# JiaxuanYou/graph-pooling

Measured on AMD Instinct MI355X. Metric: graphs/sec fwd+bwd, DD padded batch N_max=500, higher is better.
Workload: dtype f32; 1 GPU; S-DD: DD-shaped padded batch, B=20/GPU, N_max=500, F=89, H=E=20, K=50, L=3, 1 pool; graphs_per_gpu=20, global_batch=20, linkpred=False, hip_graph=True, parallelism=dp1

## Files before the change

### graph_pooling_amd/csrc/dp_common.h

```cpp
#pragma once
#include <hip/hip_runtime.h>
#include <cstddef>
#include <cstdint>
#include <cstdio>
#include <cstring>
#include <atomic>
#include <mutex>

#include "../../include/diffpool_hip.h"

namespace dp {

void set_error(const char* fmt, ...);
const char* last_error();

#define DP_CHECK_ARG(cond, ...)                      \
    do {                                             \
        if (!(cond)) {                               \
            ::dp::set_error(__VA_ARGS__);            \
            return DP_ERR_INVALID_ARG;               \
        }                                            \
    } while (0)

int* device_error_word();
// ... 413 lines not shown
    const float* x0[2];
    int x_shared;
    const float* params;
    L0Stack st[2];
    const float* Y[DP_MAX_LAYERS];
    const float* invn[DP_MAX_LAYERS];
    const float* stats[DP_MAX_LAYERS];
    const float* Z[2];
    int ldz[2];
    int coff[2][DP_MAX_LAYERS];
    int K;
    long wp_off, bp_off;
    const float* S;
    const float* Tt;
    const float* dXn;
    const float* dAn;
    const float* d_assign;
    const float* dZe;
    const unsigned short *pkA, *pkAt;
    int pk_ld;
    const int* pk_flag;
    const int* pk_sym;
    float* slabs;
    long slab_gstride;
    unsigned short* vs;
    float* part;
    float* gpart;
    int* bar;
};
bool level0_bwd_persistent_ok(const Level0Bwd& a);
size_t level0_bwd_vs_elems(const Level0Bwd& a);
size_t level0_bwd_gpart_floats(const Level0Bwd& a);
void level0_backward(Seq& q, const Level0Bwd& a);
bool level0_persistent_ok(const Level0Fwd& a);
size_t level0_bar_ints(int B);
int* level0_seq_word(int* bar);
size_t level0_xpart_floats(const Level0Fwd& a);
size_t level0_vs_elems(const Level0Fwd& a);
size_t level0_part_floats(const Level0Fwd& a);
size_t level0_mpart_floats(const Level0Fwd& a);
const int* level0_error_word(const int* bar);
void level0_forward(Seq& q, const Level0Fwd& a);

struct HeadArgs {
    const float* Z;
    int ldz, n, rw, featoff;
    int* argmax;
    int lda;
    const float* params;
    int n_pred;
    int dims[DP_MAX_PRED + 2];
    long w_off[DP_MAX_PRED + 1], b_off[DP_MAX_PRED + 1];
    float* hid[DP_MAX_PRED + 2];
    int B;
    long long* labels;
    const int* poison[DP_MAX_LEVELS + 1];
    int n_poison;
};
struct HeadBwdArgs {
    HeadArgs h;
    const float* d_ypred;
    float* grads;
    int n_levels;
    struct Level {
        float* dZ;
        const int* argmax;
        int lda, n, ldz, rw, featoff;
    } lv[DP_MAX_LEVELS + 1];
};
bool head_supported(const HeadArgs& a);
void head_fwd(Seq& q, const HeadArgs& a);
void head_bwd(Seq& q, const HeadBwdArgs& a);

bool small_level_fused_ok(int B, int n, const int* dims, int L, bool dadj);
size_t small_level_part_floats(int B, int n, int L);
void small_level_fwd(Seq& q, const SmallLevelIO& io, int B, int n, const int* dims, int L, int add_self, int bn);
struct SmallHeadFold {
    HeadBwdArgs hb;
    int level;
    int zcol;
    float* part;
};
size_t small_head_fold_part_floats(const HeadArgs& h);
bool small_head_fold_fits(int B, int n, const int* dims, int L, bool dadj, const HeadArgs& h);
void small_level_bwd(Seq& q, const SmallLevelIO& io, const float* dZe, float* dX0, float* dadj, float* slabs,
                     long slab_stride, int B, int n, const int* dims, int L, int add_self, int bn,
                     const SmallHeadFold* hf = nullptr);

void build_batch(Seq& q, const int* src, const int* dst, const int* edge_ptr, const int* label, const int* node_ptr,
                 float* adj, unsigned short* pk, unsigned short* pkt, float* feats, float* assign, int* num_nodes,
                 int* errors, int* degree, int B, int N, int F, int mode, int symmetric, int max_edges_per_graph);

void gather_labels(Seq& q, const long long* src, long long* dst, int B);

void clip_adam_step(Seq& q, float* params, float* grads, float* exp_avg, float* exp_avg_sq, long n, float max_norm,
                    float beta1, float beta2, float eps, float step_size, float inv_bc2_sqrt, float* total_norm_out,
                    int* step_counter = nullptr, float lr = 0.f);

void csr_aggregate_fwd(Seq& q, const float* table, int ldt, const int* indptr, const int* indices, float* out, int ldo,
                       int n_rows, int feat, int mean, float beta, const float* values = nullptr);
void csr_aggregate_bwd_scatter(Seq& q, const float* dout, int ldo, const int* indptr, const int* indices, float* dtable,
                               int ldt, int n_rows, int feat, int mean, const float* values = nullptr);

void segment_max_part(Seq& q, const float* Z, int ldz, const int* chunk_tab, int n_chunks, int F, float* pv, int* pi);

void set2set_prep_weights(Seq& q, const float* w_ih, const float* w_hh, float* wt, int d);

void linkpred_fwd(Seq& q, const float* S, int lds, const float* adj, const int* num_nodes, float* loss_out,
                  int B, int n, int K, const float* norm = nullptr );
void linkpred_bwd(Seq& q, const float* S, int lds, const float* adj, const int* num_nodes, const float* dloss,
                  float* dS, int ldds, int B, int n, int K, int accumulate, const float* norm = nullptr);
void linkpred_fwd_packed(Seq& q, const float* S, int lds, const unsigned short* pk, const int* num_nodes,
                         float* loss_out, int B, int n, int K, const float* norm = nullptr);
void linkpred_bwd_packed(Seq& q, const float* S, int lds, const unsigned short* pk, const unsigned short* pkt,
                         const int* num_nodes, const float* dloss, float* dS, int ldds, int B, int n, int K,
                         int accumulate, const float* norm = nullptr);

struct AssignEntPick {
    int lanes;
    int quad;
};
AssignEntPick assign_ent_pick(const void* S, int lds, const void* dS, int ldds, int K);
size_t assign_ent_part_doubles();
void assign_entropy_fwd(Seq& q, const float* S, int lds, const int* num_nodes, float weight, float* ent_out,
                        float* total_inout, int B, int n, int K);
void assign_entropy_bwd(Seq& q, const float* S, int lds, const int* num_nodes, const float* dloss, float weight,
                        float* dS, int ldds, int accumulate, int B, int n, int K);

size_t frob_link_ws_doubles(long long rows, int B, int K);
void frob_link_w_dense(Seq& q, const float* S, int lds, const void* adj, const void* adj_t, int packed, int ld,
                       const int* num_nodes, float* W, int B, int N, int K);
void frob_link_fwd(Seq& q, const float* S, int lds, const float* W, const void* adj, int adj_kind, int adj_ld,
                   const int* num_nodes, const int* node_off, const int* nnz_ptr, const float* link_norm, float wscale,
                   float* G, float* loss_out, float* total_inout, int B, int N, long long rows, int K,
                   const int* csr_indptr = nullptr );
void frob_link_bwd(Seq& q, const float* S, int lds, const float* W, const float* G, const int* num_nodes,
                   const int* node_off, const float* link_norm, const float* dloss, float wscale, float* dS, int ldds,
                   int accumulate, int B, int N, long long rows, int K);

}
```

### graph_pooling_amd/csrc/dp_model.hip

```cpp
#include "dp_common.h"

namespace dp {

void set2set_fwd(Seq& q, const float* emb, int lde, const float* w_ih, const float* w_hh, const float* b_ih,
                 const float* b_hh, const float* Wp, const float* bp, float* out, int B, int n, int d, void* save);
void set2set_bwd(Seq& q, const float* emb, int lde, const float* w_ih, const float* w_hh, const float* b_ih,
                 const float* b_hh, const float* Wp, const float* bp, const float* out, const float* dout,
                 float* demb, int ldde, float* dw_ih, float* dw_hh, float* db_ih, float* db_hh, float* dWp,
                 float* dbp, int B, int n, int d, const void* save);
size_t set2set_save_bytes(int B, int n, int d);

namespace {

struct LevelInfo {
    int j;
    int n, G, L;
    const dp_stack_cfg* e;
    const dp_stack_cfg* a;
    int D, Da, K;
    int ctot[DP_MAX_LAYERS];
    int coff_e[DP_MAX_LAYERS], coff_a[DP_MAX_LAYERS];
    int cmax;
};

// ... 1135 lines not shown
                featoff += rw;
            } else {
                set2set_bwd(q, sv.Zm, li.D, PW(params, c.s2s_off[0]), PW(params, c.s2s_off[1]), PW(params, c.s2s_off[2]),
                            PW(params, c.s2s_off[3]), PW(params, c.s2s_off[4]), PW(params, c.s2s_off[5]), sv.feat, dfeat,
                            dZm, li.D, grads + c.s2s_off[0], grads + c.s2s_off[1], grads + c.s2s_off[2],
                            grads + c.s2s_off[3], grads + c.s2s_off[4], grads + c.s2s_off[5], B, li.n, li.D, sv.s2s);
                mask_rows(q, dZm, li.D, gr[j].dZe, li.D, num_nodes, B, li.n, li.D);
            }
        }
    }
    for (int j = P; j >= 0; --j) {
        const LevelInfo& li = p.lv[j];
        const LevelSave& lv = sv.lv[j];
        const int n = li.n;
        if (p.bwd[j] == Tier::Persistent) {
            Level0Bwd f = p.l0b;
            level0_operands(f, sv, params, x, adj, assign_x);
            f.dXn = P >= 1 ? gr[1].dX0 : nullptr;
            f.dAn = P >= 1 ? gr[1].dAdj : nullptr;
            f.d_assign = d_assign;
            f.dZe = gr[0].dZe;
            f.slabs = slabs;
            f.slab_gstride = slab_stride * KS;
            f.vs = l0_vs; f.part = wh.xr.l0_bwd; f.gpart = l0_gpart;
            f.bar = wh.l0_bar;
            level0_backward(q, f);
            continue;
        }
        LevelIO io = level_io(j, sv, x, adj, assign_x, dropout, sc, pkp);
        if (j < P) {
            const int K = li.K, D = li.D;
            float *const dS = sc.dS, *const dlog = sc.dlog, *const V = sc.V, *const V2 = sc.V2;
            unsigned short* const vs = sc.vs;
            bool vsplit_used = false;
            const float* dS2 = nullptr;
            const float* dXn = gr[j + 1].dX0;
            const float* dAn = gr[j + 1].dAdj;
            {
                unsigned short* vsplit =
                    (j == 0 && pkp && aggregate_packed_usable(io.adj, n, K)) ? vs : nullptr;
                vsplit_used = vsplit != nullptr;
                GemmDesc d[4] = {
                    {lv.S, dXn, gr[j].dZe, nullptr, n, D, K, K, D, D, (long)n * K, (long)K * D, (long)n * D, false, false,
                     1.f, 1.f, 0},
                    {lv.Ze, dXn, dS, nullptr, n, K, D, D, D, K, (long)n * D, (long)K * D, (long)n * K, false, true, 1.f,
                     0.f, 0},
                    {lv.S, dAn, V, nullptr, n, K, K, K, K, K, (long)n * K, (long)K * K, (long)n * K, false, true, 1.f, 0.f,
                     0, 0, 0, vsplit, (K + 15) / 16, ((n + 31) / 32) * 4, 0},
                    {lv.S, dAn, V2, nullptr, n, K, K, K, K, K, (long)n * K, (long)K * K, (long)n * K, false, false, 1.f,
                     0.f, 0}};
                if (!gr[j].dAdj) {
                    d[3] = GemmDesc{lv.T, dAn, V2, nullptr, n, K, K, K, K, K, (long)n * K, (long)K * K, (long)n * K, false,
                                    false, 1.f, 0.f, 0};
                    dS2 = V2;
                }
                bgemm_group(q, d, 4, B);
            }
            if (gr[j].dAdj)
                bgemm(q, lv.T, dAn, dS, nullptr, B, n, K, K, K, K, K, (long)n * K, (long)K * K, (long)n * K, false, false,
                      1.f, 1.f, 0);
            aggregate(q, io.adj, V, K, dS, K, B, n, K, false, 1.f, j == 0 ? pkp : nullptr, vs, vsplit_used);
            if (gr[j].dAdj)
                bgemm(q, V2, lv.S, gr[j].dAdj, nullptr, B, n, n, K, K, K, n, (long)n * K, (long)n * K, (long)n * n, false,
                      true, 1.f, 1.f, 0);
            if (j == 0 && d_assign) axpy(q, dS, d_assign, 1.f, (long)B * n * K);
            softmax_mask_bwd(q, lv.S, K, dS, K, j == 0 ? num_nodes : nullptr, dlog, K, B, n, K,
                             c.assign_pred_b_off[j] >= 0 ? slabs + c.assign_pred_b_off[j] : nullptr, slab_stride * KS,
                             dS2);
            {
                const int ksn = n >= 256 ? KS : 1;
                GemmDesc d2[2] = {
                    {dlog, lv.Za, slabs + c.assign_pred_w_off[j], nullptr, K, li.Da, n, K, li.Da, li.Da, (long)n * K,
                     (long)n * li.Da, slab_stride * KS, true, false, 1.f, 0.f, 0, slab_stride, 0},
                    {dlog, PW(params, c.assign_pred_w_off[j]), gr[j].dZa, nullptr, n, li.Da, K, K, li.Da, li.Da,
                     (long)n * K, 0, (long)n * li.Da, false, false, 1.f, 0.f, 0, 0, 0, nullptr, 0, 0, 0, 1}};
                bgemm_group(q, d2, 2, B, ksn);
            }
        }
        io.bar = bz.bar + 64 * j;
        io.gr = &gr[j];
        io.hf = fold && j == P ? &hf : nullptr;
        level_backward(q, p, j, lv, io, params, sc);
    }
    reduce_slabs(q, slabs, slab_stride, B * KS, grads, c.n_graph_params, 0);
    return q.err;
}

size_t encoder_save_bytes(const dp_encoder_cfg& c) { return layout_save(encoder_plan(c, false), nullptr).total; }

int encoder_save_locate(const dp_encoder_cfg& c, int level, int field, size_t* offset, size_t* count) {
    char* const base = reinterpret_cast<char*>(size_t(1) << 20);
    const EncoderPlan plan = encoder_plan(c, false);
    SaveLayout sv = layout_save(plan, base);
    const LevelInfo& li = plan.lv[level];
    const LevelSave& lv = sv.lv[level];
    const size_t B = c.B;
    const void* p = nullptr;
    size_t cnt = 0;
    switch (field) {
        case DP_SAVE_ARGMAX: p = lv.argmax; cnt = B * readout_width(c, li); break;
        case DP_SAVE_S: p = lv.S; cnt = B * li.n * li.K; break;
        case DP_SAVE_XPOOL: p = lv.Xn; cnt = B * li.K * li.D; break;
        case DP_SAVE_ADJPOOL: p = lv.An; cnt = B * li.K * li.K; break;
        case DP_SAVE_Z: p = lv.Ze; cnt = B * li.n * li.D; break;
        case DP_SAVE_ZASSIGN: p = lv.Za; cnt = B * li.n * li.Da; break;
        default: set_error("dp_encoder_save_locate: unknown field %d", field); return DP_ERR_INVALID_ARG;
    }
    if (!p) {
        set_error("dp_encoder_save_locate: level %d has no field %d", level, field);
        return DP_ERR_INVALID_ARG;
    }
    *offset = (size_t)(static_cast<const char*>(p) - base);
    *count = cnt;
    return DP_OK;
}

int encoder_validate(const dp_encoder_cfg* c) { return validate(c); }

}
```

### graph_pooling_amd/csrc/dp_rowops.hip

```cpp
#include "dp_common.h"

namespace dp {

#define L2_EPS 1e-12f
#define BN_EPS 1e-5f

typedef float f4u __attribute__((ext_vector_type(4), aligned(4)));

__device__ inline float team_sum(float v) {
    return row16_sum(v);
}
__device__ inline float team_max(float v) {
    return row16_max(v);
}

static inline bool row_quads_ok(const RowGroups& g) {
    if (knobs().no_row_quads) return false;
    for (int i = 0; i < g.G; ++i)
        if (g.w[i] < 4 || (g.w[i] & 3)) return false;
    return true;
}
static inline int team_grid(long items) {
    long blocks = (items + 15) / 16;
    if (blocks > 4096) blocks = 4096;
// ... 1800 lines not shown
void relu_bwd_inplace(Seq& q, float* d, const float* h, long count) {
    if (!q.ok() || count <= 0) return;
    hipLaunchKernelGGL(k_relu_bwd, dim3((count + 255) / 256), dim3(256), 0, q.stream, d, h, count);
    q.check_launch("relu_bwd");
}

__global__ void k_axpy(float* y, const float* x, float a, long count) {
    const long i = (long)blockIdx.x * blockDim.x + threadIdx.x;
    if (i < count) y[i] += a * x[i];
}
void axpy(Seq& q, float* y, const float* x, float a, long count) {
    if (!q.ok() || count <= 0) return;
    hipLaunchKernelGGL(k_axpy, dim3((count + 255) / 256), dim3(256), 0, q.stream, y, x, a, count);
    q.check_launch("axpy");
}

__global__ __launch_bounds__(256) void k_ce_fwd(const float* logits, const long long* label, float* loss,
                                                float* prob, int B, int C, float* also_zero, float* dunit) {
    __shared__ float red[256];
    float acc = 0.f;
    for (int b = threadIdx.x; b < B; b += 256) {
        const float* l = logits + (long)b * C;
        float m = -INFINITY;
        for (int c = 0; c < C; ++c) m = fmaxf(m, l[c]);
        float s = 0.f;
        for (int c = 0; c < C; ++c) s += expf(l[c] - m);
        const float lse = m + logf(s);
        const long long y = label[b];
        acc += lse - l[y];
        if (prob)
            for (int c = 0; c < C; ++c) prob[(long)b * C + c] = expf(l[c] - lse);
        if (dunit)
            for (int c = 0; c < C; ++c)
                dunit[(long)b * C + c] = (expf(l[c] - lse) - (y == c ? 1.f : 0.f)) / (float)B;
    }
    red[threadIdx.x] = acc;
    __syncthreads();
    for (int s = 128; s > 0; s >>= 1) {
        if (threadIdx.x < s) red[threadIdx.x] += red[threadIdx.x + s];
        __syncthreads();
    }
    if (threadIdx.x == 0) {
        loss[0] = red[0] / (float)B;
        if (also_zero) also_zero[0] = 0.f;
    }
}
void ce_fwd(Seq& q, const float* logits, const long long* label, float* loss, float* prob, int B, int C,
            float* also_zero, float* dunit) {
    if (!q.ok()) return;
    hipLaunchKernelGGL(k_ce_fwd, dim3(1), dim3(256), 0, q.stream, logits, label, loss, prob, B, C, also_zero, dunit);
    q.check_launch("ce_fwd");
}
__global__ void k_ce_bwd(const float* prob, const long long* label, const float* dloss, float scale, float* dl,
                         int B, int C) {
    const int i = blockIdx.x * blockDim.x + threadIdx.x;
    if (i >= B * C) return;
    const int b = i / C, c = i % C;
    const float g = (dloss ? dloss[0] : 1.f) * scale / (float)B;
    dl[i] = g * (prob[i] - (label[b] == c ? 1.f : 0.f));
}
void ce_bwd(Seq& q, const float* prob, const long long* label, const float* dloss, float scale, float* dlogits,
            int B, int C) {
    if (!q.ok()) return;
    hipLaunchKernelGGL(k_ce_bwd, dim3((B * C + 255) / 256), dim3(256), 0, q.stream, prob, label, dloss, scale,
                       dlogits, B, C);
    q.check_launch("ce_bwd");
}

__global__ void k_argmax_rows(const float* X, int ldx, long long* out, int rows, int cols) {
    const int r = blockIdx.x * blockDim.x + threadIdx.x;
    if (r >= rows) return;
    const float* x = X + (long)r * ldx;
    int best = 0;
    for (int c = 1; c < cols; ++c)
        if (x[c] > x[best]) best = c;
    out[r] = best;
}
void argmax_rows(Seq& q, const float* X, int ldx, long long* out, int rows, int cols) {
    if (!q.ok() || rows <= 0) return;
    hipLaunchKernelGGL(k_argmax_rows, dim3((rows + 255) / 256), dim3(256), 0, q.stream, X, ldx, out, rows, cols);
    q.check_launch("argmax_rows");
}

__global__ __launch_bounds__(1024) void k_reduce_slabs(const float* slabs, long stride, int B, float* out,
                                                       long count, int accumulate) {
    __shared__ float red[16][64];
    const int cl = threadIdx.x & 63, rl = threadIdx.x >> 6;
    const long i = (long)blockIdx.x * 64 + cl;
    float s = 0.f;
    if (i < count)
        for (int b = rl; b < B; b += 16) s += slabs[(long)b * stride + i];
    red[rl][cl] = s;
    __syncthreads();
    if (rl == 0 && i < count) {
        float t = 0.f;
#pragma unroll
        for (int k = 0; k < 16; ++k) t += red[k][cl];
        out[i] = accumulate ? out[i] + t : t;
    }
}
void reduce_slabs(Seq& q, const float* slabs, long stride, int B, float* out, long count, int accumulate) {
    if (!q.ok() || count <= 0) return;
    hipLaunchKernelGGL(k_reduce_slabs, dim3((count + 63) / 64), dim3(1024), 0, q.stream, slabs, stride, B, out, count,
                       accumulate);
    q.check_launch("reduce_slabs");
}

}
```

### graph_pooling_amd/csrc/dp_small.hip

```cpp
#include "dp_common.h"

namespace dp {

#define SM_L2_EPS 1e-12f
#define SM_BN_EPS 1e-5f

#ifdef DP_STAMP
__device__ unsigned long long g_small_stamps[2][32];
#define SM_STAMP(k, i)                                                                       \
    do {                                                                                     \
        if (blockIdx.x == 0 && threadIdx.x == 0) g_small_stamps[k][i] = __builtin_amdgcn_s_memtime(); \
    } while (0)
#else
#define SM_STAMP(k, i) \
    do {               \
    } while (0)
#endif

namespace {

__device__ inline float sm_team_sum(float v) {
    return row16_sum(v);
}

// ... 547 lines not shown
                if (tl == 0) sc_st16(part_l, (unsigned)(((long)r * a.B + b) * 16), sc_tagged(mean, m2, (seq << 4) | (unsigned)(l + 1)));
            }
        }
        SM_STAMP(0, 12 + 6 * l);
        if (last) break;
        if (stats) {
            SM_STAMP(0, 13 + 6 * l);
            for (int r = team; r < n; r += NTEAMS) {
                float pm[SM_BMAX16], pq[SM_BMAX16];
                const bool ok = sm_poll_row(part_l, (unsigned)((long)r * a.B * 16), a.B, bn_tag, pm, pq, a.spin_limit, a.bar,
                                            a.dev_err);
                float sm = 0.f;
#pragma unroll
                for (int u = 0; u < SM_BMAX16; ++u) sm += (tl + 16 * u < a.B) ? pm[u] : 0.f;
                float m = sm_team_sum(sm) / (float)a.B;
                float s2 = 0.f;
#pragma unroll
                for (int u = 0; u < SM_BMAX16; ++u) {
                    const float d = pm[u] - m;
                    s2 += (tl + 16 * u < a.B) ? pq[u] + (float)dout * d * d : 0.f;
                }
                float rstd = 1.0f / sqrtf(sm_team_sum(s2) / ((float)a.B * (float)dout) + SM_BN_EPS);
                if (!ok) m = rstd = __builtin_nanf("");
                if (tl == 0) {
                    if (b == 0) {
                        a.stats[l][r * 2] = m;
                        a.stats[l][r * 2 + 1] = rstd;
                    }
                    mu[r] = m;
                    rs[r] = rstd;
                }
            }
            SM_STAMP(0, 14 + 6 * l);
        } else {
            for (int r = tid; r < n; r += NT) {
                mu[r] = 0.f;
                rs[r] = 1.f;
            }
        }
        lds_barrier();
        for (int r = team; r < n; r += NTEAMS)
            for (int k = tl; k < dout; k += 16) {
                const float v = (fmaxf(U[r * dout + k], 0.f) - mu[r]) * rs[r];
                X[r * dout + k] = v;
                a.Ze[((long)b * n + r) * a.ldz + a.coff[l] + k] = v;
            }
        lds_barrier();
        SM_STAMP(0, 15 + 6 * l);
        wo += din * dout;
        bo += dout;
    }
    sm_finish(a.bar, a.seq, seq, a.B);
}

struct SmallLevelBwdArgs {
    const float* adj;
    const float* x0;
    int ldx0;
    const float* params;
    long w_off[DP_MAX_LAYERS], b_off[DP_MAX_LAYERS];
    int dims[DP_MAX_LAYERS + 1];
    int L;
    const float* Y[DP_MAX_LAYERS];
    int ldY[DP_MAX_LAYERS];
    const float* invn[DP_MAX_LAYERS];
    const float* stats[DP_MAX_LAYERS];
    const float* Ze;
    int ldz;
    int coff[DP_MAX_LAYERS];
    const float* dZe;
    float* dX0;
    float* dadj;
    float* slabs;
    long slab_stride;
    float* part;
    int* bar;
    int* seq;
    int* dev_err;
    int spin_limit, target_bias;
    int B, n, add_self, bn;
    int omax, wtot, D;
    SmDiv qd0, qD;
    SmDiv qdout[DP_MAX_LAYERS];
    int fold, hlevel, zcol, htot;
    HeadBwdArgs hb;
    float* hpart;
};

struct SmHead {
    int nP, d0, d1, C, wup, hup, E;
    __host__ __device__ SmHead(const HeadArgs& h) : nP(h.n_pred), d0(h.dims[0]), d1(h.dims[1]), C(h.dims[h.n_pred]) {
        wup = hup = 0;
        for (int i = 1; i < nP; ++i) {
            wup += h.dims[i] * h.dims[i + 1];
            hup += h.dims[i];
        }
        E = (hup + 1) / 2;
    }
    __host__ __device__ size_t lds_floats(int B) const {
        return (size_t)d1 * d0 + wup + 2 * (size_t)B * hup + (size_t)B * d0 + (size_t)B * C;
    }
};
constexpr unsigned SM_HEAD_TAG = 15u;

__global__ __launch_bounds__(1024) void k_small_level_bwd(SmallLevelBwdArgs a) {
    extern __shared__ __attribute__((aligned(16))) float lds[];
    const int b = blockIdx.x, tid = threadIdx.x;
    const int n = a.n, L = a.L, D = a.D, d0 = a.dims[0];
    const unsigned seq = (unsigned)a.seq[0];
    float* A = lds;
    float* DA = A + n * n;
    float* X0 = DA + (a.dadj ? n * n : 0);
    float* ZE = X0 + n * d0;
    float* DZ = ZE + n * D;
    float* YS = DZ + n * D;
    float* WL = YS + (L - 1) * n * a.omax;
    float* IV = WL + a.wtot;
    float* RS = IV + L * n;
    float* dU = RS + L * n;
    float* G = dU + n * a.omax;
    float* P = G + n * a.omax;
    float* M0 = P + n * a.omax;
    float* M1 = M0 + n;
    float* DB = M1 + n;
    float* DBW = DB + a.omax;
    const int tl = tid & 15, team = tid >> 4;
    const int NT = blockDim.x, NTEAMS = blockDim.x >> 4;
    const SmHead hz(a.hb.h);
    const int B = a.B;
    float* HW0 = DBW + 16 * a.omax;
    float* HWU = HW0 + hz.d1 * hz.d0;
    float* HH = HWU + hz.wup;
    float* HG = HH + B * hz.hup;
    float* HF = HG + B * hz.hup;
    float* HY = HF + B * hz.d0;
    SM_STAMP(1, 16);
    int win = -1;
    if (a.fold) {
        if (tid < hz.d0) {
            for (int lv = 0; lv < a.hb.n_levels; ++lv) {
                const int f = tid - a.hb.lv[lv].featoff;
                if (f >= 0 && f < a.hb.lv[lv].rw) win = a.hb.lv[lv].argmax[(long)b * a.hb.lv[lv].lda + f];
            }
        }
        const HeadArgs& h = a.hb.h;
        sm_dma(HY, B * hz.C, [&](int e) { return a.hb.d_ypred + e; });
        sm_dma(HW0, hz.d1 * hz.d0, [&](int e) { return h.params + h.w_off[0] + e; });
        int wo = 0, ho = 0;
        for (int i = 1; i < hz.nP; ++i) {
            const int cnt = h.dims[i] * h.dims[i + 1];
            sm_dma(HWU + wo, cnt, [&](int e) { return h.params + h.w_off[i] + e; });
            sm_dma(HH + ho, B * h.dims[i], [&](int e) { return h.hid[i] + e; });
            wo += cnt;
            ho += B * h.dims[i];
        }
        sm_dma(HF, B * hz.d0, [&](int e) { return h.hid[0] + e; });
    }

    sm_dma(A, n * n, [&](int e) { return a.adj + (long)b * n * n + e; });
    sm_dma(X0, n * d0, [&](int e) { return a.x0 + ((long)b * n + a.qd0.quot(e)) * a.ldx0 + a.qd0.rem(e); });
    sm_dma(ZE, n * D, [&](int e) { return a.Ze + ((long)b * n + a.qD.quot(e)) * a.ldz + a.qD.rem(e); });
    sm_dma(DZ, n * D, [&](int e) { return a.dZe + ((long)b * n + a.qD.quot(e)) * a.ldz + a.qD.rem(e); });
    {
        int wo = 0;
        for (int l = 0; l < L; ++l) {
            const int din = a.dims[l], dout = a.dims[l + 1];
            const float* w = a.params + a.w_off[l];
            sm_dma(WL + wo, din * dout, [&](int e) { return w + e; });
            wo += din * dout;
            const float* iv = a.invn[l] + (long)b * n;
            sm_dma(IV + l * n, n, [&](int e) { return iv + e; });
            if (l < L - 1) {
                const float* y = a.Y[l];
                const int ldy = a.ldY[l];
                const SmDiv q = a.qdout[l];
                sm_dma(YS + l * n * a.omax, n * dout, [&](int e) { return y + ((long)b * n + q.quot(e)) * ldy + q.rem(e); });
                if (a.bn) {
                    const float* st = a.stats[l];
                    sm_dma(RS + l * n, n, [&](int e) { return st + e * 2 + 1; });
                }
            }
        }
    }
    if (a.dadj)
        for (int i = tid; i < n * n; i += NT) DA[i] = 0.f;
    SM_STAMP(1, 17);
    __syncthreads();
    SM_STAMP(1, 18);

    if (a.fold) {
        const HeadArgs& h = a.hb.h;
        int ho = B * hz.hup, wo = hz.wup;
        for (int i = hz.nP - 1; i >= 1; --i) {
            const int din = h.dims[i], dout = h.dims[i + 1];
            wo -= din * dout;
            ho -= B * din;
            const float* go = i == hz.nP - 1 ? HY + b * dout : HG + ho + B * din + b * dout;
            const float* W = HWU + wo;
            for (int k = tid; k < din; k += NT) {
                float s = 0.f;
#pragma unroll 8
                for (int j = 0; j < dout; ++j) s += go[j] * W[j * din + k];
                HG[ho + b * din + k] = HH[ho + b * din + k] > 0.f ? s : 0.f;
            }
            __syncthreads();
        }
        const ScBuf hp = sc_buf(a.hpart, (size_t)B * hz.E * 16);
        for (int e = tid; e < hz.E; e += NT) {
            float v[2] = {0.f, 0.f};
            for (int u = 0; u < 2; ++u) {
                int t = 2 * e + u, blk = 0;
                for (int i = 1; i < hz.nP && t >= 0; ++i) {
                    if (t < h.dims[i]) v[u] = HG[blk + b * h.dims[i] + t];
                    t -= h.dims[i];
                    blk += B * h.dims[i];
                }
            }
            sc_st16(hp, (unsigned)(((long)b * hz.E + e) * 16), sc_tagged(v[0], v[1], (seq << 4) | SM_HEAD_TAG));
        }
        const float* g1 = hz.nP == 1 ? HY + b * hz.C : HG + b * hz.d1;
        for (int k = tid, it = 0; k < hz.d0; k += NT, ++it) {
            float s = 0.f;
#pragma unroll 8
            for (int j = 0; j < hz.d1; ++j) s += g1[j] * HW0[j * hz.d0 + k];
            for (int lv = 0; lv < a.hb.n_levels; ++lv) {
                const HeadBwdArgs::Level& t = a.hb.lv[lv];
                const int f = k - t.featoff;
                if (f >= 0 && f < t.rw) {
                    const int r = it == 0 ? win : t.argmax[(long)b * t.lda + f];
                    if (r < 0) continue;
                    if (lv == a.hlevel) DZ[r * D + a.zcol + f] += s;
                    else t.dZ[((long)b * t.n + r) * t.ldz + f] = s;
                }
            }
        }
        SM_STAMP(1, 19);
    }

    u32x4 hprobe = (u32x4){0u, 0u, 0u, 0u};
    const unsigned htag = ((seq << 4) | SM_HEAD_TAG) ^ (a.target_bias ? 0x40000000u : 0u);
    int wo_end = a.wtot;
    for (int l = L - 1; l >= 0; --l) {
        const int din = a.dims[l], dout = a.dims[l + 1];
        const bool last = l == L - 1;
        const bool has_bn = !last && a.bn;
        const bool has_relu = !last;
        wo_end -= din * dout;
        const float* W = WL + wo_end;
        const float* Xl = l == 0 ? X0 : ZE + a.coff[l - 1];
        const int ldx = l == 0 ? d0 : D;
        const float* Yl = last ? ZE + a.coff[l] : YS + l * n * a.omax;
        const int ldy = last ? D : dout;
        float* dx = DZ + a.coff[l];
        for (int i = tid; i < 16 * dout; i += NT) DBW[i] = 0.f;
        if (has_bn) {
            const ScBuf part_l = sc_buf(a.part + (long)l * a.B * n * 4, (size_t)a.B * n * 16);
            const unsigned bn_tag = (seq << 4) | (unsigned)(l + 1);
            const float* xh = ZE + a.coff[l];
            for (int r = team; r < n; r += NTEAMS) {
                float s0 = 0.f, s1 = 0.f;
                for (int c = tl; c < dout; c += 16) {
                    const float d = dx[r * D + c];
                    s0 += d;
                    s1 += d * xh[r * D + c];
                }
                s0 = sm_team_sum(s0);
                s1 = sm_team_sum(s1);
                if (tl == 0) sc_st16(part_l, (unsigned)(((long)r * a.B + b) * 16), sc_tagged(s0, s1, bn_tag));
            }
            for (int r = team; r < n; r += NTEAMS) {
                float p0[SM_BMAX16], p1[SM_BMAX16];
                const bool ok = sm_poll_row(part_l, (unsigned)((long)r * a.B * 16), a.B,
                                            bn_tag ^ (a.target_bias ? 0x40000000u : 0u), p0, p1, a.spin_limit, a.bar, a.dev_err);
                float s0 = 0.f, s1 = 0.f;
#pragma unroll
                for (int u = 0; u < SM_BMAX16; ++u) {
                    s0 += (tl + 16 * u < a.B) ? p0[u] : 0.f;
                    s1 += (tl + 16 * u < a.B) ? p1[u] : 0.f;
                }
                s0 = sm_team_sum(s0);
                s1 = sm_team_sum(s1);
                const float cnt = (float)a.B * (float)dout;
                if (tl == 0) {
                    M0[r] = ok ? s0 / cnt : __builtin_nanf("");
                    M1[r] = s1 / cnt;
                }
            }
        }
        if (a.fold && l == 0 && tid < B * hz.E) hprobe = sc_ld16(sc_buf(a.hpart, (size_t)B * hz.E * 16), (unsigned)tid * 16u);
        lds_barrier();
        float* dbb = a.b_off[l] >= 0 ? a.slabs + (long)b * a.slab_stride + a.b_off[l] : nullptr;
        for (int r0 = 0; r0 < n; r0 += NTEAMS) {
            const int r = min(r0 + team, n - 1);
            const bool valid = r0 + team < n;
            const float rstd = has_bn ? RS[l * n + r] : 1.f;
            const float m0 = has_bn ? M0[r] : 0.f, m1 = has_bn ? M1[r] : 0.f;
            const float inv = IV[l * n + r];
            const bool project = inv < 1.0f / SM_L2_EPS;
            float dot = 0.f;
            float dv[4];
#pragma unroll
            for (int k = 0; k < 4; ++k) {
                const int c = tl + 16 * k;
                float d = 0.f;
                if (c < dout) {
                    d = dx[r * D + c];
                    const float yy = Yl[r * ldy + c];
                    if (has_bn) d = rstd * (d - m0 - ZE[r * D + a.coff[l] + c] * m1);
                    if (has_relu) d = yy > 0.f ? d : 0.f;
                    dot += d * yy;
                }
                dv[k] = d;
            }
            dot = sm_team_sum(dot);
#pragma unroll
            for (int k = 0; k < 4; ++k) {
                const int c = tl + 16 * k;
                float v = 0.f;
                if (c < dout && valid) {
                    v = project ? inv * (dv[k] - Yl[r * ldy + c] * dot) : inv * dv[k];
                    dU[r * dout + c] = v;
                }
                if (dbb && 16 * k < dout) {
                    v += __shfl_xor(v, 16, 64);
                    v += __shfl_xor(v, 32, 64);
                    if ((tid & 63) < 16 && c < dout) DBW[(tid >> 6) * dout + c] += v;
                }
            }
        }
        lds_barrier();
        if (dbb)
            for (int c = tid; c < dout; c += NT) {
                float t = 0.f;
#pragma unroll
                for (int w = 0; w < 16; ++w) t += DBW[w * dout + c];
                dbb[c] = t;
            }
        lds_mma2<true, false>(A, n, dU, dout, n, dout, n, [&](int m, int c, float v) {
            G[m * dout + c] = a.add_self ? v + dU[m * dout + c] : v;
        });
        if (a.dadj)
            lds_mma2<false, false>(Xl, ldx, W, dout, n, dout, din, [&](int m, int c, float v) { P[m * dout + c] = v; },
                                  ((n + 15) / 16) * ((dout + 15) / 16));
        lds_barrier();
        {
            float* dWb = a.slabs + (long)b * a.slab_stride + a.w_off[l];
            lds_mma2<true, false>(Xl, ldx, G, dout, din, dout, n, [&](int k, int c, float v) { dWb[k * dout + c] = v; });
        }
        if (l > 0) {
            float* dxin = DZ + a.coff[l - 1];
            lds_mma2<false, true>(G, dout, W, dout, n, din, dout, [&](int r, int k, float v) { dxin[r * D + k] += v; },
                                 1);
        } else if (a.dX0) {
            lds_mma2<false, true>(G, dout, W, dout, n, din, dout, [&](int r, int k, float v) {
                a.dX0[((long)b * n + r) * d0 + k] = v;
            }, 1);
        }
        if (a.dadj)
            lds_mma2<false, true>(dU, dout, P, dout, n, n, dout, [&](int r, int m, float v) { DA[r * n + m] += v; }, 2);
        lds_barrier();
    }
    if (a.dadj)
        for (int i = tid; i < n * n; i += NT) a.dadj[(long)b * n * n + i] = DA[i];
    SM_STAMP(1, 20);
    if (a.fold) {
        const HeadArgs& h = a.hb.h;
        const ScBuf hp = sc_buf(a.hpart, (size_t)B * hz.E * 16);
        bool ok = true;
        for (int t = tid; t < B * hz.E; t += NT) {
            const int bb = t / hz.E, e = t - bb * hz.E;
            u32x4 q = hprobe;
            for (int it = 0;; ++it) {
                if (t != tid || it > 0) q = sc_ld16(hp, (unsigned)t * 16u);
                if (q[1] == htag && q[3] == htag) break;
                if (it > a.spin_limit) {
                    __hip_atomic_store(a.bar + 1, 1, __ATOMIC_RELAXED, __HIP_MEMORY_SCOPE_AGENT);
                    dev_err_raise(a.dev_err, DP_DEVERR_BARRIER);
                    ok = false;
                    break;
                }
                if (t != tid || it > 0) __builtin_amdgcn_s_sleep(2);
            }
            for (int u = 0; u < 2; ++u) {
                int x = 2 * e + u, blk = 0;
                for (int i = 1; i < hz.nP && x >= 0; ++i) {
                    if (x < h.dims[i]) HG[blk + bb * h.dims[i] + x] = __uint_as_float(q[2 * u]);
                    x -= h.dims[i];
                    blk += B * h.dims[i];
                }
            }
        }
        ok = __syncthreads_and(ok);
        SM_STAMP(1, 21);
        const int lo = a.htot * b / B, hi = a.htot * (b + 1) / B;
        for (int e = lo + tid; e < hi; e += NT) {
            int i = 0, r = e, ho = 0;
            for (; i < hz.nP - 1; ++i) {
                const int seg = h.dims[i + 1] * (h.dims[i] + (h.b_off[i] >= 0 ? 1 : 0));
                if (r < seg) break;
                r -= seg;
                if (i > 0) ho += B * h.dims[i];
            }
            const int din = h.dims[i], dout = h.dims[i + 1];
            const float* go = i == hz.nP - 1 ? HY : HG + (i > 0 ? ho + B * din : 0);
            const float* hin = i == 0 ? HF : HH + ho;
            float s = 0.f;
            if (r < dout * din) {
                const int j = r / din, k = r - j * din;
#pragma unroll 8
                for (int bb = 0; bb < B; ++bb) s += go[bb * dout + j] * hin[bb * din + k];
                a.hb.grads[h.w_off[i] + r] = ok ? s : __builtin_nanf("");
            } else {
                const int j = r - dout * din;
#pragma unroll 8
                for (int bb = 0; bb < B; ++bb) s += go[bb * dout + j];
                a.hb.grads[h.b_off[i] + j] = ok ? s : __builtin_nanf("");
            }
        }
        SM_STAMP(1, 22);
    }
    sm_finish(a.bar, a.seq, seq, a.B);
}

size_t small_lds_floats_fwd(int B, int n, int din, int dout) {
    return (size_t)n * n + (size_t)n * din + (size_t)din * dout + 2 * (size_t)n * dout + 2 * n + dout +
           (size_t)B * n * 2 + 16;
}
size_t small_lds_floats_bwd(int B, int n, int din, int dout) {
    return 2 * (size_t)n * n + 2 * (size_t)n * din + (size_t)din * dout + 4 * (size_t)n * dout + 4 * n + 17 * (size_t)dout +
           (size_t)B * n * 2 + 16;
}

}

bool small_level_supported(int B, int n, int din, int dout) {
    if (n > 64 || din > 256 || dout > 256) return false;
    const size_t f = small_lds_floats_fwd(B, n, din, dout), bw = small_lds_floats_bwd(B, n, din, dout);
    return (f > bw ? f : bw) * sizeof(float) <= 150 * 1024;
}

static void small_attr(Seq& q) {
    static DynLdsOnce fwd, bwd;
    ensure_dyn_lds(q, fwd, reinterpret_cast<const void*>(&k_small_gcn_fwd), 160 * 1024, "k_small_gcn_fwd");
    ensure_dyn_lds(q, bwd, reinterpret_cast<const void*>(&k_small_gcn_bwd), 160 * 1024, "k_small_gcn_bwd");
}

void small_gcn_fwd(Seq& q, const float* adj, const float* x0, int ldx0, const float* yprev, int ldyp,
                   const float* part_prev, float* stats_prev, float* xout, int ldxo, const float* W, const float* bias,
                   float* y, int ldy, float* invn, float* part, int B, int n, int din, int dout, int add_self,
                   int stats) {
    if (!q.ok()) return;
    small_attr(q);
    if (!q.ok()) return;
    SmallFwdArgs a{adj, x0, ldx0, yprev, ldyp, part_prev, stats_prev, xout, ldxo, W, bias, y, ldy, invn, part,
                   B, n, din, dout, add_self, stats, sm_div(din)};
    hipLaunchKernelGGL(k_small_gcn_fwd, dim3(B), dim3(1024), small_lds_floats_fwd(B, n, din, dout) * sizeof(float),
                       q.stream, a);
    q.check_launch("small_gcn_fwd");
}

void small_gcn_bwd(Seq& q, const float* adj, const float* xin, int ldxin, const float* W, const float* y, int ldy,
                   const float* xhat, int ldxh, const float* invn, const float* stats, const float* part2,
                   const float* dx, int lddx, float* dxin, int lddxin, float* part2_prev, float* dadj, float* dW,
                   float* db, long slab_stride, int B, int n, int din, int dout, int add_self, int has_bn,
                   int has_relu) {
    if (!q.ok()) return;
    small_attr(q);
    if (!q.ok()) return;
    SmallBwdArgs a{adj, xin, ldxin, W, y, ldy, xhat, ldxh, invn, stats, part2, dx, lddx, dxin, lddxin, part2_prev,
                   dadj, dW, db, slab_stride, B, n, din, dout, add_self, has_bn, has_relu, sm_div(din), sm_div(dout)};
    hipLaunchKernelGGL(k_small_gcn_bwd, dim3(B), dim3(1024), small_lds_floats_bwd(B, n, din, dout) * sizeof(float),
                       q.stream, a);
    q.check_launch("small_gcn_bwd");
}


static size_t small_level_lds_fwd(int B, int n, const int* dims, int L) {
    int dmax = 0, omax = 0, wtot = 0, btot = 0;
    for (int l = 0; l < L; ++l) {
        dmax = dims[l] > dmax ? dims[l] : dmax;
        omax = dims[l + 1] > omax ? dims[l + 1] : omax;
        wtot += dims[l] * dims[l + 1];
        btot += dims[l + 1];
    }
    return (size_t)n * n + (size_t)n * dmax + 2 * (size_t)n * omax + 2 * n + wtot + btot + 64 + 16;
}
static size_t small_level_lds_bwd(int B, int n, const int* dims, int L, bool dadj) {
    int omax = 0, wtot = 0, D = 0;
    for (int l = 0; l < L; ++l) {
        omax = dims[l + 1] > omax ? dims[l + 1] : omax;
        wtot += dims[l] * dims[l + 1];
        D += dims[l + 1];
    }
    return (size_t)n * n * (dadj ? 2 : 1) + (size_t)n * dims[0] + 2 * (size_t)n * D + (size_t)(L - 1) * n * omax + wtot +
           2 * (size_t)L * n + 3 * (size_t)n * omax + 2 * n + 17 * (size_t)omax + 64 + 16;
}
static int device_cus() {
    static std::atomic<int> cus[64];
    int dev = 0;
    if (hipGetDevice(&dev) != hipSuccess || dev < 0 || dev >= 64) return 0;
    int v = cus[dev].load(std::memory_order_relaxed);
    if (v == 0) {
        hipDeviceProp_t prop;
        v = hipGetDeviceProperties(&prop, dev) == hipSuccess ? prop.multiProcessorCount : -1;
        cus[dev].store(v, std::memory_order_relaxed);
    }
    return v > 0 ? v : 0;
}
static bool level_kernels_admitted() {
    static std::atomic<int> state[64];
    int dev = 0;
    if (hipGetDevice(&dev) != hipSuccess || dev < 0 || dev >= 64) return false;
    int v = state[dev].load(std::memory_order_relaxed);
    if (v == 0) {
        v = 1;
        const void* fns[2] = {reinterpret_cast<const void*>(&k_small_level_fwd),
                              reinterpret_cast<const void*>(&k_small_level_bwd)};
        for (const void* fn : fns) {
            int blocks = 0;
            hipError_t e = hipFuncSetAttribute(fn, hipFuncAttributeMaxDynamicSharedMemorySize, 159 * 1024);
            if (e == hipSuccess) e = hipOccupancyMaxActiveBlocksPerMultiprocessor(&blocks, fn, 1024, 150 * 1024);
            if (e != hipSuccess || blocks < 1) {
                (void)hipGetLastError();
                set_error("whole-level kernels disabled: the runtime admits %d resident 1024-thread workgroups with 150 KiB "
                          "of LDS per CU (%s)", blocks, hipGetErrorString(e));
                v = -1;
            }
        }
        state[dev].store(v, std::memory_order_relaxed);
    }
    return v > 0;
}
bool small_level_fused_ok(int B, int n, const int* dims, int L, bool dadj) {
    if (knobs().no_level_fusion || L < 2 || L > DP_MAX_LAYERS || n > 64) return false;
    for (int l = 0; l <= L; ++l)
        if (dims[l] > 256 || (l > 0 && dims[l] > 64)) return false;
    if (small_level_lds_fwd(B, n, dims, L) * sizeof(float) > 150 * 1024) return false;
    if (small_level_lds_bwd(B, n, dims, L, dadj) * sizeof(float) > 150 * 1024) return false;
    const int cus = device_cus();
    return cus > 0 && B <= cus / 2 && B <= 16 * SM_BMAX16 && level_kernels_admitted();
}
size_t small_level_part_floats(int B, int n, int L) { return (size_t)(L > 1 ? L - 1 : 1) * B * n * 4; }
static int head_grad_entries(const HeadArgs& h) {
    int tot = 0;
    for (int i = 0; i < h.n_pred; ++i) tot += h.dims[i + 1] * (h.dims[i] + (h.b_off[i] >= 0 ? 1 : 0));
    return tot;
}
size_t small_head_fold_part_floats(const HeadArgs& h) {
    const SmHead z(h);
    return (size_t)h.B * (z.E > 0 ? z.E : 1) * 4;
}
bool small_head_fold_fits(int B, int n, const int* dims, int L, bool dadj, const HeadArgs& h) {
    if (h.n_pred < 1 || h.B != B || (long)head_grad_entries(h) * B >= (1L << 31)) return false;
    return (small_level_lds_bwd(B, n, dims, L, dadj) + SmHead(h).lds_floats(B)) * sizeof(float) <= 150 * 1024;
}

void small_level_fwd(Seq& q, const SmallLevelIO& io, int B, int n, const int* dims, int L, int add_self, int bn) {
    if (!q.ok()) return;
    static DynLdsOnce attr;
    ensure_dyn_lds(q, attr, reinterpret_cast<const void*>(&k_small_level_fwd), 159 * 1024, "k_small_level_fwd");
    if (!q.ok()) return;
    SmallLevelFwdArgs a{};
    a.adj = io.adj; a.x0 = io.x0; a.ldx0 = io.ldx0; a.params = io.params; a.L = L;
    a.Ze = io.Ze; a.ldz = io.ldz; a.part = io.part; a.bar = io.bar; a.seq = q.seq_word;
    a.B = B; a.n = n; a.add_self = add_self; a.bn = bn;
    for (int l = 0; l <= L; ++l) a.dims[l] = dims[l];
    for (int l = 0; l < L; ++l) {
        a.w_off[l] = io.w_off[l]; a.b_off[l] = io.b_off[l];
        a.Y[l] = io.Y[l]; a.ldY[l] = io.ldY[l]; a.invn[l] = io.invn[l]; a.stats[l] = io.stats[l];
        a.coff[l] = io.coff[l];
        a.dmax = dims[l] > a.dmax ? dims[l] : a.dmax;
        a.omax = dims[l + 1] > a.omax ? dims[l + 1] : a.omax;
        a.wtot += dims[l] * dims[l + 1];
        a.btot += dims[l + 1];
    }
    a.qd0 = sm_div(dims[0]);
    a.dev_err = device_error_word();
    a.spin_limit = knobs().test_barrier_fail ? 64 : SM_SPIN_LIMIT;
    a.target_bias = knobs().test_barrier_fail ? 1 : 0;
    hipLaunchKernelGGL(k_small_level_fwd, dim3(B), dim3(1024), small_level_lds_fwd(B, n, dims, L) * sizeof(float),
                       q.stream, a);
    q.check_launch("small_level_fwd");
}

void small_level_bwd(Seq& q, const SmallLevelIO& io, const float* dZe, float* dX0, float* dadj, float* slabs,
                     long slab_stride, int B, int n, const int* dims, int L, int add_self, int bn,
                     const SmallHeadFold* hf) {
    if (!q.ok()) return;
    static DynLdsOnce attr;
    ensure_dyn_lds(q, attr, reinterpret_cast<const void*>(&k_small_level_bwd), 159 * 1024, "k_small_level_bwd");
    if (!q.ok()) return;
    SmallLevelBwdArgs a{};
    a.adj = io.adj; a.x0 = io.x0; a.ldx0 = io.ldx0; a.params = io.params; a.L = L;
    a.Ze = io.Ze; a.ldz = io.ldz; a.part = io.part; a.bar = io.bar; a.seq = q.seq_word;
    a.dZe = dZe; a.dX0 = dX0; a.dadj = dadj; a.slabs = slabs; a.slab_stride = slab_stride;
    a.B = B; a.n = n; a.add_self = add_self; a.bn = bn;
    for (int l = 0; l <= L; ++l) a.dims[l] = dims[l];
    for (int l = 0; l < L; ++l) {
        a.w_off[l] = io.w_off[l]; a.b_off[l] = io.b_off[l];
        a.Y[l] = io.Y[l]; a.ldY[l] = io.ldY[l]; a.invn[l] = io.invn[l]; a.stats[l] = io.stats[l];
        a.coff[l] = io.coff[l];
        a.omax = dims[l + 1] > a.omax ? dims[l + 1] : a.omax;
        a.wtot += dims[l] * dims[l + 1];
        a.D += dims[l + 1];
        a.qdout[l] = sm_div(dims[l + 1]);
    }
    a.qd0 = sm_div(dims[0]);
    a.qD = sm_div(a.D);
    a.dev_err = device_error_word();
    a.spin_limit = knobs().test_barrier_fail ? 64 : SM_SPIN_LIMIT;
    a.target_bias = knobs().test_barrier_fail ? 1 : 0;
    size_t lds = small_level_lds_bwd(B, n, dims, L, dadj != nullptr);
    if (hf) {
        a.fold = 1;
        a.hb = hf->hb;
        a.hlevel = hf->level;
        a.zcol = hf->zcol;
        a.hpart = hf->part;
        a.htot = head_grad_entries(hf->hb.h);
        lds += SmHead(hf->hb.h).lds_floats(B);
    }
    hipLaunchKernelGGL(k_small_level_bwd, dim3(B), dim3(1024), lds * sizeof(float), q.stream, a);
    q.check_launch("small_level_bwd");
}

#ifdef DP_STAMP
extern "C" __attribute__((visibility("default"))) int dp_debug_stamps(unsigned long long* out) {
    return (int)hipMemcpyFromSymbol(out, HIP_SYMBOL(g_small_stamps), sizeof(unsigned long long) * 64);
}
#endif

}
```

Baseline: 85420 graphs/s.

## Move head weight-gradient reduction from fused level kernel into slab-reduce kernel

The fused small-level backward kernel used to exchange per-graph head hidden gradients through tagged scratch with cross-block spin-waiting, then reduce the head weight and bias gradients over the batch inside each block. Now each block only writes its own hidden gradients to a plain buffer. The batch reduction of head gradients runs in extra workgroups appended to the final reduce_slabs launch. This removes the inter-block handshake and shrinks per-block LDS, since only one graph's head data is staged. The cost is a somewhat heavier reduce kernel that re-reads hidden activations from global memory.

```diff
diff --git a/graph_pooling_amd/csrc/dp_common.h b/graph_pooling_amd/csrc/dp_common.h
--- a/graph_pooling_amd/csrc/dp_common.h
+++ b/graph_pooling_amd/csrc/dp_common.h
@@ -519,6 +519,9 @@
     float* part;
 };
 size_t small_head_fold_part_floats(const HeadArgs& h);
+long head_grad_entries(const HeadArgs& h);
+void reduce_slabs_head(Seq& q, const float* slabs, long stride, int B, float* out, long count,
+                       const SmallHeadFold& hf);
 bool small_head_fold_fits(int B, int n, const int* dims, int L, bool dadj, const HeadArgs& h);
 void small_level_bwd(Seq& q, const SmallLevelIO& io, const float* dZe, float* dX0, float* dadj, float* slabs,
                      long slab_stride, int B, int n, const int* dims, int L, int add_self, int bn,
diff --git a/graph_pooling_amd/csrc/dp_model.hip b/graph_pooling_amd/csrc/dp_model.hip
--- a/graph_pooling_amd/csrc/dp_model.hip
+++ b/graph_pooling_amd/csrc/dp_model.hip
@@ -1241,7 +1241,8 @@
         io.hf = fold && j == P ? &hf : nullptr;
         level_backward(q, p, j, lv, io, params, sc);
     }
-    reduce_slabs(q, slabs, slab_stride, B * KS, grads, c.n_graph_params, 0);
+    if (fold) reduce_slabs_head(q, slabs, slab_stride, B * KS, grads, c.n_graph_params, hf);
+    else reduce_slabs(q, slabs, slab_stride, B * KS, grads, c.n_graph_params, 0);
     return q.err;
 }
 
diff --git a/graph_pooling_amd/csrc/dp_rowops.hip b/graph_pooling_amd/csrc/dp_rowops.hip
--- a/graph_pooling_amd/csrc/dp_rowops.hip
+++ b/graph_pooling_amd/csrc/dp_rowops.hip
@@ -1906,9 +1906,80 @@
     q.check_launch("argmax_rows");
 }
 
-__global__ __launch_bounds__(1024) void k_reduce_slabs(const float* slabs, long stride, int B, float* out,
-                                                       long count, int accumulate) {
-    __shared__ float red[16][64];
+struct HeadGradArgs {
+    int tiles;
+    int n_pred, B, hup;
+    int htot;
+    int dims[DP_MAX_PRED + 2];
+    long w_off[DP_MAX_PRED + 1], b_off[DP_MAX_PRED + 1];
+    const float* hid[DP_MAX_PRED + 1];
+    const float* d_ypred;
+    const float* hgrad;
+    float* grads;
+};
+constexpr int HG_CHUNK = 32;
+constexpr int HG_THREADS = 128;
+
+__device__ inline void head_grad_entry(const HeadGradArgs& a, int e) {
+    int i = 0, r = e, rem = e, goff = 0, gcol = 0;
+    int din = a.dims[0], dout = a.dims[1];
+    long woff = a.w_off[0], boff = a.b_off[0];
+    const float* hin = a.hid[0];
+    bool found = false;
+#pragma unroll
+    for (int t = 0; t < DP_MAX_PRED + 1; ++t) {
+        if (t < a.n_pred) {
+            const int seg = a.dims[t + 1] * (a.dims[t] + (a.b_off[t] >= 0 ? 1 : 0));
+            if (!found && (rem < seg || t == a.n_pred - 1)) {
+                i = t; r = rem; goff = gcol;
+                din = a.dims[t]; dout = a.dims[t + 1];
+                woff = a.w_off[t]; boff = a.b_off[t];
+                hin = a.hid[t];
+                found = true;
+            }
+            rem -= seg;
+            gcol += a.dims[t + 1];
+        }
+    }
+    const int B = a.B;
+    const bool weight = r < dout * din;
+    const int j = weight ? r / din : r - dout * din;
+    const int k = weight ? r - j * din : 0;
+    const bool top = i == a.n_pred - 1;
+    const float* gp = (top ? a.d_ypred : a.hgrad + goff) + j;
+    const int gs = top ? dout : a.hup;
+    const float* xp = hin + (weight ? k : 0);
+    const int xs = weight ? din : 0;
+    float s = 0.f;
+    for (int b0 = 0; b0 < B; b0 += HG_CHUNK) {
+        float g[HG_CHUNK], x[HG_CHUNK];
+#pragma unroll
+        for (int u0 = 0; u0 < HG_CHUNK; u0 += 8) {
+            if (b0 + u0 < B) {
+#pragma unroll
+                for (int u = u0; u < u0 + 8; ++u) {
+                    const long row = min(b0 + u, B - 1);
+                    g[u] = gp[row * gs];
+                    x[u] = xp[row * xs];
+                }
+            }
+        }
+        if (weight) {
+#pragma unroll
+            for (int u = 0; u < HG_CHUNK; ++u)
+                if (b0 + u < B) s += g[u] * x[u];
+        } else {
+#pragma unroll
+            for (int u = 0; u < HG_CHUNK; ++u)
+                if (b0 + u < B) s += g[u];
+        }
+    }
+    if (weight) a.grads[woff + r] = s;
+    else a.grads[boff + j] = s;
+}
+
+__device__ inline void reduce_slab_tile(const float* slabs, long stride, int B, float* out, long count, int accumulate,
+                                        float (&red)[16][64]) {
     const int cl = threadIdx.x & 63, rl = threadIdx.x >> 6;
     const long i = (long)blockIdx.x * 64 + cl;
     float s = 0.f;
@@ -1923,11 +1994,50 @@
         out[i] = accumulate ? out[i] + t : t;
     }
 }
+__global__ __launch_bounds__(1024) void k_reduce_slabs(const float* slabs, long stride, int B, float* out,
+                                                       long count, int accumulate) {
+    __shared__ float red[16][64];
+    reduce_slab_tile(slabs, stride, B, out, count, accumulate, red);
+}
+__global__ __launch_bounds__(1024) void k_reduce_slabs_head(const float* slabs, long stride, int B, float* out,
+                                                            long count, HeadGradArgs hg) {
+    __shared__ float red[16][64];
+    if ((int)blockIdx.x >= hg.tiles) {
+        const int e = ((int)blockIdx.x - hg.tiles) * HG_THREADS + threadIdx.x;
+        if (threadIdx.x < HG_THREADS && e < hg.htot) head_grad_entry(hg, e);
+        return;
+    }
+    reduce_slab_tile(slabs, stride, B, out, count, 0, red);
+}
 void reduce_slabs(Seq& q, const float* slabs, long stride, int B, float* out, long count, int accumulate) {
     if (!q.ok() || count <= 0) return;
     hipLaunchKernelGGL(k_reduce_slabs, dim3((count + 63) / 64), dim3(1024), 0, q.stream, slabs, stride, B, out, count,
                        accumulate);
     q.check_launch("reduce_slabs");
 }
-
-}
+void reduce_slabs_head(Seq& q, const float* slabs, long stride, int B, float* out, long count,
+                       const SmallHeadFold& hf) {
+    if (!q.ok()) return;
+    const HeadArgs& h = hf.hb.h;
+    HeadGradArgs hg{};
+    hg.tiles = count > 0 ? (int)((count + 63) / 64) : 0;
+    hg.n_pred = h.n_pred;
+    hg.B = h.B;
+    hg.htot = (int)head_grad_entries(h);
+    for (int i = 0; i <= h.n_pred; ++i) hg.dims[i] = h.dims[i];
+    for (int i = 0; i < h.n_pred; ++i) {
+        hg.w_off[i] = h.w_off[i];
+        hg.b_off[i] = h.b_off[i];
+        hg.hid[i] = h.hid[i];
+        if (i >= 1) hg.hup += h.dims[i];
+    }
+    hg.d_ypred = hf.hb.d_ypred;
+    hg.hgrad = hf.part;
+    hg.grads = hf.hb.grads;
+    const int head_wgs = (hg.htot + HG_THREADS - 1) / HG_THREADS;
+    hipLaunchKernelGGL(k_reduce_slabs_head, dim3(hg.tiles + head_wgs), dim3(1024), 0, q.stream, slabs, stride, B, out,
+                       count, hg);
+    q.check_launch("reduce_slabs_head");
+}
+
+}
diff --git a/graph_pooling_amd/csrc/dp_small.hip b/graph_pooling_amd/csrc/dp_small.hip
--- a/graph_pooling_amd/csrc/dp_small.hip
+++ b/graph_pooling_amd/csrc/dp_small.hip
@@ -653,26 +653,22 @@
     int omax, wtot, D;
     SmDiv qd0, qD;
     SmDiv qdout[DP_MAX_LAYERS];
-    int fold, hlevel, zcol, htot;
+    int fold, hlevel, zcol;
     HeadBwdArgs hb;
-    float* hpart;
+    float* hgrad;
 };
 
 struct SmHead {
-    int nP, d0, d1, C, wup, hup, E;
+    int nP, d0, d1, C, wup, hup;
     __host__ __device__ SmHead(const HeadArgs& h) : nP(h.n_pred), d0(h.dims[0]), d1(h.dims[1]), C(h.dims[h.n_pred]) {
         wup = hup = 0;
         for (int i = 1; i < nP; ++i) {
             wup += h.dims[i] * h.dims[i + 1];
             hup += h.dims[i];
         }
-        E = (hup + 1) / 2;
-    }
-    __host__ __device__ size_t lds_floats(int B) const {
-        return (size_t)d1 * d0 + wup + 2 * (size_t)B * hup + (size_t)B * d0 + (size_t)B * C;
-    }
+    }
+    __host__ __device__ size_t lds_floats() const { return (size_t)d1 * d0 + wup + 2 * (size_t)hup + (size_t)C; }
 };
-constexpr unsigned SM_HEAD_TAG = 15u;
 
 __global__ __launch_bounds__(1024) void k_small_level_bwd(SmallLevelBwdArgs a) {
     extern __shared__ __attribute__((aligned(16))) float lds[];
@@ -698,13 +694,11 @@
     const int tl = tid & 15, team = tid >> 4;
     const int NT = blockDim.x, NTEAMS = blockDim.x >> 4;
     const SmHead hz(a.hb.h);
-    const int B = a.B;
     float* HW0 = DBW + 16 * a.omax;
     float* HWU = HW0 + hz.d1 * hz.d0;
     float* HH = HWU + hz.wup;
-    float* HG = HH + B * hz.hup;
-    float* HF = HG + B * hz.hup;
-    float* HY = HF + B * hz.d0;
+    float* HG = HH + hz.hup;
+    float* HY = HG + hz.hup;
     SM_STAMP(1, 16);
     int win = -1;
     if (a.fold) {
@@ -715,17 +709,16 @@
             }
         }
         const HeadArgs& h = a.hb.h;
-        sm_dma(HY, B * hz.C, [&](int e) { return a.hb.d_ypred + e; });
+        sm_dma(HY, hz.C, [&](int e) { return a.hb.d_ypred + (long)b * hz.C + e; });
         sm_dma(HW0, hz.d1 * hz.d0, [&](int e) { return h.params + h.w_off[0] + e; });
         int wo = 0, ho = 0;
         for (int i = 1; i < hz.nP; ++i) {
             const int cnt = h.dims[i] * h.dims[i + 1];
             sm_dma(HWU + wo, cnt, [&](int e) { return h.params + h.w_off[i] + e; });
-            sm_dma(HH + ho, B * h.dims[i], [&](int e) { return h.hid[i] + e; });
+            sm_dma(HH + ho, h.dims[i], [&](int e) { return h.hid[i] + (long)b * h.dims[i] + e; });
             wo += cnt;
-            ho += B * h.dims[i];
-        }
-        sm_dma(HF, B * hz.d0, [&](int e) { return h.hid[0] + e; });
+            ho += h.dims[i];
+        }
     }
 
     sm_dma(A, n * n, [&](int e) { return a.adj + (long)b * n * n + e; });
@@ -761,35 +754,23 @@
 
     if (a.fold) {
         const HeadArgs& h = a.hb.h;
-        int ho = B * hz.hup, wo = hz.wup;
+        int ho = hz.hup, wo = hz.wup;
         for (int i = hz.nP - 1; i >= 1; --i) {
             const int din = h.dims[i], dout = h.dims[i + 1];
             wo -= din * dout;
-            ho -= B * din;
-            const float* go = i == hz.nP - 1 ? HY + b * dout : HG + ho + B * din + b * dout;
+            ho -= din;
+            const float* go = i == hz.nP - 1 ? HY : HG + ho + din;
             const float* W = HWU + wo;
             for (int k = tid; k < din; k += NT) {
                 float s = 0.f;
 #pragma unroll 8
                 for (int j = 0; j < dout; ++j) s += go[j] * W[j * din + k];
-                HG[ho + b * din + k] = HH[ho + b * din + k] > 0.f ? s : 0.f;
+                HG[ho + k] = HH[ho + k] > 0.f ? s : 0.f;
             }
             __syncthreads();
         }
-        const ScBuf hp = sc_buf(a.hpart, (size_t)B * hz.E * 16);
-        for (int e = tid; e < hz.E; e += NT) {
-            float v[2] = {0.f, 0.f};
-            for (int u = 0; u < 2; ++u) {
-                int t = 2 * e + u, blk = 0;
-                for (int i = 1; i < hz.nP && t >= 0; ++i) {
-                    if (t < h.dims[i]) v[u] = HG[blk + b * h.dims[i] + t];
-                    t -= h.dims[i];
-                    blk += B * h.dims[i];
-                }
-            }
-            sc_st16(hp, (unsigned)(((long)b * hz.E + e) * 16), sc_tagged(v[0], v[1], (seq << 4) | SM_HEAD_TAG));
-        }
-        const float* g1 = hz.nP == 1 ? HY + b * hz.C : HG + b * hz.d1;
+        for (int e = tid; e < hz.hup; e += NT) a.hgrad[(long)b * hz.hup + e] = HG[e];
+        const float* g1 = hz.nP == 1 ? HY : HG;
         for (int k = tid, it = 0; k < hz.d0; k += NT, ++it) {
             float s = 0.f;
 #pragma unroll 8
@@ -808,8 +789,6 @@
         SM_STAMP(1, 19);
     }
 
-    u32x4 hprobe = (u32x4){0u, 0u, 0u, 0u};
-    const unsigned htag = ((seq << 4) | SM_HEAD_TAG) ^ (a.target_bias ? 0x40000000u : 0u);
     int wo_end = a.wtot;
     for (int l = L - 1; l >= 0; --l) {
         const int din = a.dims[l], dout = a.dims[l + 1];
@@ -858,7 +837,6 @@
                 }
             }
         }
-        if (a.fold && l == 0 && tid < B * hz.E) hprobe = sc_ld16(sc_buf(a.hpart, (size_t)B * hz.E * 16), (unsigned)tid * 16u);
         lds_barrier();
         float* dbb = a.b_off[l] >= 0 ? a.slabs + (long)b * a.slab_stride + a.b_off[l] : nullptr;
         for (int r0 = 0; r0 < n; r0 += NTEAMS) {
@@ -934,62 +912,6 @@
     if (a.dadj)
         for (int i = tid; i < n * n; i += NT) a.dadj[(long)b * n * n + i] = DA[i];
     SM_STAMP(1, 20);
-    if (a.fold) {
-        const HeadArgs& h = a.hb.h;
-        const ScBuf hp = sc_buf(a.hpart, (size_t)B * hz.E * 16);
-        bool ok = true;
-        for (int t = tid; t < B * hz.E; t += NT) {
-            const int bb = t / hz.E, e = t - bb * hz.E;
-            u32x4 q = hprobe;
-            for (int it = 0;; ++it) {
-                if (t != tid || it > 0) q = sc_ld16(hp, (unsigned)t * 16u);
-                if (q[1] == htag && q[3] == htag) break;
-                if (it > a.spin_limit) {
-                    __hip_atomic_store(a.bar + 1, 1, __ATOMIC_RELAXED, __HIP_MEMORY_SCOPE_AGENT);
-                    dev_err_raise(a.dev_err, DP_DEVERR_BARRIER);
-                    ok = false;
-                    break;
-                }
-                if (t != tid || it > 0) __builtin_amdgcn_s_sleep(2);
-            }
-            for (int u = 0; u < 2; ++u) {
-                int x = 2 * e + u, blk = 0;
-                for (int i = 1; i < hz.nP && x >= 0; ++i) {
-                    if (x < h.dims[i]) HG[blk + bb * h.dims[i] + x] = __uint_as_float(q[2 * u]);
-                    x -= h.dims[i];
-                    blk += B * h.dims[i];
-                }
-            }
-        }
-        ok = __syncthreads_and(ok);
-        SM_STAMP(1, 21);
-        const int lo = a.htot * b / B, hi = a.htot * (b + 1) / B;
-        for (int e = lo + tid; e < hi; e += NT) {
-            int i = 0, r = e, ho = 0;
-            for (; i < hz.nP - 1; ++i) {
-                const int seg = h.dims[i + 1] * (h.dims[i] + (h.b_off[i] >= 0 ? 1 : 0));
-                if (r < seg) break;
-                r -= seg;
-                if (i > 0) ho += B * h.dims[i];
-            }
-            const int din = h.dims[i], dout = h.dims[i + 1];
-            const float* go = i == hz.nP - 1 ? HY : HG + (i > 0 ? ho + B * din : 0);
-            const float* hin = i == 0 ? HF : HH + ho;
-            float s = 0.f;
-            if (r < dout * din) {
-                const int j = r / din, k = r - j * din;
-#pragma unroll 8
-                for (int bb = 0; bb < B; ++bb) s += go[bb * dout + j] * hin[bb * din + k];
-                a.hb.grads[h.w_off[i] + r] = ok ? s : __builtin_nanf("");
-            } else {
-                const int j = r - dout * din;
-#pragma unroll 8
-                for (int bb = 0; bb < B; ++bb) s += go[bb * dout + j];
-                a.hb.grads[h.b_off[i] + j] = ok ? s : __builtin_nanf("");
-            }
-        }
-        SM_STAMP(1, 22);
-    }
     sm_finish(a.bar, a.seq, seq, a.B);
 }
 
@@ -1112,18 +1034,18 @@
     return cus > 0 && B <= cus / 2 && B <= 16 * SM_BMAX16 && level_kernels_admitted();
 }
 size_t small_level_part_floats(int B, int n, int L) { return (size_t)(L > 1 ? L - 1 : 1) * B * n * 4; }
-static int head_grad_entries(const HeadArgs& h) {
-    int tot = 0;
-    for (int i = 0; i < h.n_pred; ++i) tot += h.dims[i + 1] * (h.dims[i] + (h.b_off[i] >= 0 ? 1 : 0));
+long head_grad_entries(const HeadArgs& h) {
+    long tot = 0;
+    for (int i = 0; i < h.n_pred; ++i) tot += (long)h.dims[i + 1] * (h.dims[i] + (h.b_off[i] >= 0 ? 1 : 0));
     return tot;
 }
 size_t small_head_fold_part_floats(const HeadArgs& h) {
     const SmHead z(h);
-    return (size_t)h.B * (z.E > 0 ? z.E : 1) * 4;
+    return (size_t)h.B * (z.hup > 0 ? z.hup : 1);
 }
 bool small_head_fold_fits(int B, int n, const int* dims, int L, bool dadj, const HeadArgs& h) {
-    if (h.n_pred < 1 || h.B != B || (long)head_grad_entries(h) * B >= (1L << 31)) return false;
-    return (small_level_lds_bwd(B, n, dims, L, dadj) + SmHead(h).lds_floats(B)) * sizeof(float) <= 150 * 1024;
+    if (h.n_pred < 1 || h.B != B || head_grad_entries(h) >= (1L << 30)) return false;
+    return (small_level_lds_bwd(B, n, dims, L, dadj) + SmHead(h).lds_floats()) * sizeof(float) <= 150 * 1024;
 }
 
 void small_level_fwd(Seq& q, const SmallLevelIO& io, int B, int n, const int* dims, int L, int add_self, int bn) {
@@ -1187,9 +1109,8 @@
         a.hb = hf->hb;
         a.hlevel = hf->level;
         a.zcol = hf->zcol;
-        a.hpart = hf->part;
-        a.htot = head_grad_entries(hf->hb.h);
-        lds += SmHead(hf->hb.h).lds_floats(B);
+        a.hgrad = hf->part;
+        lds += SmHead(hf->hb.h).lds_floats();
     }
     hipLaunchKernelGGL(k_small_level_bwd, dim3(B), dim3(1024), lds * sizeof(float), q.stream, a);
     q.check_launch("small_level_bwd");
```

After: 86380 graphs/s (median of 6 runs). +1.1%, better.
